# libjxl/jxl-rs

Measured on AMD Instinct MI355X. Metric: megapixels/sec decoded (8K VarDCT d1 reconstruction: dequant+CfL+IDCT+LF smoothing+Gaborish+EPF), higher is better.
Workload: dtype f32

## Files before the change

### jxl_rs_amd/csrc/k_filters_fused.hip

```cpp
#include "jxlh_internal.h"
#include "run_plan.h"

#ifndef JXLH_FUSED_TH
#define JXLH_FUSED_TH 56
#endif
#ifndef JXLH_FUSED_THREADS
#define JXLH_FUSED_THREADS 512
#endif
#ifndef JXLH_FUSED_TH_LOW
#define JXLH_FUSED_TH_LOW 24
#endif
#ifndef JXLH_FUSED_THREADS_LOW
#define JXLH_FUSED_THREADS_LOW 256
#endif
#ifndef JXLH_FUSED_WAVES_PER_EU
#define JXLH_FUSED_WAVES_PER_EU 6
#endif
#ifndef JXLH_FUSED_E0_WPE
#define JXLH_FUSED_E0_WPE 3
#endif
#ifndef JXLH_FUSED_E0_THREADS
#define JXLH_FUSED_E0_THREADS 128
#endif
#ifndef JXLH_SPARSE_MAX
#define JXLH_SPARSE_MAX 64
#endif
#ifndef JXLH_DENSE_ITEMS
#define JXLH_DENSE_ITEMS 40
#endif
#ifndef JXLH_DENSE_ITEMS0
#define JXLH_DENSE_ITEMS0 40
#endif

#ifndef JXLH_NT_FLOAD
#define JXLH_NT_FLOAD false
#endif
#ifndef JXLH_NT_FSTORE
#define JXLH_NT_FSTORE false
#endif
namespace jxlh {
namespace {

struct FusedArgs {
  const float* in[3];
  float* out[3];
  const float* inv_sigma;
  uint32_t stride, sigma_stride;
  int w, h;
  int y0, y1;
  float gab_k[3][3];
  float scale[3];
  float sm0, bsm0, sm1, bsm1, sm2, bsm2;
  int tiled_in, xblocks;
};

__device__ __forceinline__ uint32_t in_offset(const FusedArgs& a, int fx, int fy) {
  return 4u * (a.tiled_in ? ((uint32_t)((fy >> 3) * a.xblocks + (fx >> 3)) * 64u +
                             (uint32_t)((fy & 4) * 8 + (fx & 7) * 4 + (fy & 3)))
                          : ((uint32_t)fy * a.stride + (uint32_t)fx));
}
template <class T>
__device__ __forceinline__ const T& at_bytes(const float* base, uint32_t byte_off) {
  return *reinterpret_cast<const T*>(reinterpret_cast<const char*>(base) + byte_off);
}
template <class T>
__device__ __forceinline__ T& at_bytes(float* base, uint32_t byte_off) {
  return *reinterpret_cast<T*>(reinterpret_cast<char*>(base) + byte_off);
}

__device__ __forceinline__ float dpp_from_left(float v) {
  return __builtin_bit_cast(float, __builtin_amdgcn_update_dpp(0, __builtin_bit_cast(int, v), 0x111, 0xf, 0xf, true));
}
__device__ __forceinline__ float dpp_from_right(float v) {
  return __builtin_bit_cast(float, __builtin_amdgcn_update_dpp(0, __builtin_bit_cast(int, v), 0x101, 0xf, 0xf, true));
}

namespace tall {
#define JXLH_TILE_TH JXLH_FUSED_TH
#define JXLH_TILE_THREADS JXLH_FUSED_THREADS
#include "k_filters_fused_tile.inc"
#undef JXLH_TILE_TH
#undef JXLH_TILE_THREADS
}
namespace low {
#define JXLH_TILE_TH JXLH_FUSED_TH_LOW
#define JXLH_TILE_THREADS JXLH_FUSED_THREADS_LOW
#include "k_filters_fused_tile.inc"
#undef JXLH_TILE_TH
#undef JXLH_TILE_THREADS
}
using tall::recip_weight_sum;

__global__ void k_selftest_recip(uint32_t lo_bits, uint32_t hi_bits, unsigned long long* mismatches) {
  const uint32_t stride = gridDim.x * blockDim.x;
  unsigned long long bad = 0;
  for (uint64_t b = (uint64_t)lo_bits + blockIdx.x * blockDim.x + threadIdx.x; b < hi_bits; b += stride) {
    const float w = __builtin_bit_cast(float, (uint32_t)b);
    const float fast = recip_weight_sum(w);
    const float ref = 1.0f / w;
    bad += __builtin_bit_cast(uint32_t, fast) != __builtin_bit_cast(uint32_t, ref);
  }
  if (bad) atomicAdd(mismatches, bad);
}

}

void launch_selftest_recip(hipStream_t s, uint32_t lo_bits, uint32_t hi_bits, unsigned long long* mismatches) {
  hipLaunchKernelGGL(k_selftest_recip, dim3(2048), dim3(256), 0, s, lo_bits, hi_bits, mismatches);
}

int launch_fused_filters(hipStream_t s, const FrameDev& f, int y0, int y1) {
  const bool gab = f.gab != 0, e0 = f.epf_iters >= 3, e1 = f.epf_iters >= 1, e2 = f.epf_iters >= 2;
  const int where = StageList{gab, f.epf_iters, false}.fused_where();
  if (where == 0 || y1 <= y0) return where;
  FusedArgs a;
  for (int c = 0; c < 3; c++) {
    a.in[c] = f.planes[c];
    a.out[c] = f.tmp[c];
    a.scale[c] = f.epf_channel_scale[c];
    for (int k = 0; k < 3; k++) a.gab_k[c][k] = f.gab_k[c][k];
  }
  a.inv_sigma = f.inv_sigma;
  a.stride = (uint32_t)f.plane_stride;
  a.sigma_stride = (uint32_t)f.xblocks;
  a.w = f.xsize;
  a.h = f.ysize;
  a.y0 = y0;
  a.y1 = y1;
  a.sm0 = f.epf_sm[0];
  a.bsm0 = f.epf_bsm[0];
  a.sm1 = f.epf_sm[1];
  a.bsm1 = f.epf_bsm[1];
  a.sm2 = f.epf_sm[2];
  a.bsm2 = f.epf_bsm[2];
  a.tiled_in = f.tiled;
  a.xblocks = f.xblocks;
  if (e0) {
    a.y0 = max(0, y0 - 4);
    a.y1 = min(f.ysize, y1 + 3);
    if (gab) low::launch_variant<true, true, false, false>(s, a);
    else low::launch_variant<false, true, false, false>(s, a);
    for (int c = 0; c < 3; c++) {
      a.in[c] = f.tmp[c];
      a.out[c] = f.planes[c];
    }
    a.tiled_in = 0;
    a.y0 = y0;
    a.y1 = y1;
    tall::launch_variant<false, false, true, true>(s, a);
    return where;
  }
  if (gab && e1 && e2) low::launch_variant<true, false, true, true>(s, a);
  else if (gab && e1) low::launch_variant<true, false, true, false>(s, a);
  else if (gab) tall::launch_variant<true, false, false, false>(s, a);
  else if (e1 && e2) low::launch_variant<false, false, true, true>(s, a);
  else low::launch_variant<false, false, true, false>(s, a);
  return where;
}

}
```

### jxl_rs_amd/csrc/k_filters_fused_tile.inc

```
constexpr int kTW = 56, kTH = JXLH_TILE_TH, kB = 4;
constexpr int kBW = kTW + 2 * kB;
constexpr int kBH = kTH + 2 * kB;
constexpr int kStrips = kBW / 4;
constexpr int kPlane = kBW * kBH;
constexpr int kThreadsDefault = JXLH_TILE_THREADS;
static_assert(kStrips == 16, "lane <-> strip mapping relies on 16-lane DPP rows");
static_assert(kTH % 4 == 0 && kThreadsDefault % 64 == 0, "tiled staging fetches 4-row groups");
constexpr int kSigW = kBW / 8 + 2, kSigH = kBH / 8 + 2;
constexpr int kDenseItems = JXLH_DENSE_ITEMS, kDenseItems0 = JXLH_DENSE_ITEMS0, kSparseMax = JXLH_SPARSE_MAX;
static_assert(kSparseMax <= 64, "a compacting wavefront takes 64 strips");

#include "filters_core.inc"

template <int kT>
__device__ __forceinline__ void mirror_fill(float* __restrict__ buf, int m, int tx0, int ty0, int w, int h, int tid) {
  const int rw = kTW + 2 * m, rh = kTH + 2 * m;
  for (int idx = tid; idx < rw * rh; idx += kT) {
    const int bx = kB - m + idx % rw, by = kB - m + idx / rw;
    const int fx = tx0 - kB + bx, fy = ty0 - kB + by;
    if (fx >= 0 && fx < w && fy >= 0 && fy < h) continue;
    const int sx = mirror(fx, w) - (tx0 - kB), sy = mirror(fy, h) - (ty0 - kB);
    if (sx < 0 || sx >= kBW || sy < 0 || sy >= kBH) continue;
#pragma unroll
    for (int c = 0; c < 3; c++) buf[c * kPlane + by * kBW + bx] = buf[c * kPlane + sy * kBW + sx];
  }
}

template <bool E0>
constexpr int fused_threads() { return E0 ? JXLH_FUSED_E0_THREADS : kThreadsDefault; }

template <bool GAB, bool E0, bool E1, bool E2>
__global__ __launch_bounds__(fused_threads<E0>(), E0 ? JXLH_FUSED_E0_WPE : JXLH_FUSED_WAVES_PER_EU) void k23_fused_filters(const FusedArgs a) {
  constexpr int kT = fused_threads<E0>();
  __shared__ __attribute__((aligned(16))) float s_buf[3 * kPlane];
  __shared__ float s_sigma[kSigH * kSigW];
  __shared__ uint16_t s_list[(kTH + 2 * kB) * kStrips];
  __shared__ int s_cnt, s_nsw;
  const int tid_kernel = threadIdx.x, tid = tid_kernel;
  const int tiles_x = (a.w + kTW - 1) / kTW;
  const int tiles_y = (a.y1 - a.y0 + kTH - 1) / kTH;
  const int b = blockIdx.x, k = b & 7, j = b >> 3;
  const int tile_y = (j / tiles_x) * 8 + k, tile_x = j % tiles_x;
  if (tile_y >= tiles_y) return;
  constexpr int kBorder = (GAB ? 1 : 0) + (E0 ? 3 : 0) + (E1 ? 2 : 0) + (E2 ? 1 : 0);
  static_assert(kBorder >= 1 && kBorder <= kB, "at least one stage");
  static_assert(!(E0 && (E1 || E2)), "EPF0 closes its kernel; EPF1/EPF2 follow in a second launch");
  const int tx0 = tile_x * kTW;
  const int ty0 = a.y0 + tile_y * kTH;
  const bool edge = tx0 - kB < 0 || ty0 - kB < 0 || tx0 + kTW + kB > a.w || ty0 + kTH + kB > a.h;
  if (tid_kernel == 0) {
    s_cnt = 0;
    s_nsw = 0;
  }

  const int sbx0 = max(tx0 - kB, 0) >> 3, sby0 = max(ty0 - kB, 0) >> 3;
  if constexpr (E0 || E1 || E2) {
    if (tid < kSigH * kSigW) {
      const int sx = min(sbx0 + tid % kSigW, (a.w - 1) >> 3), sy = min(sby0 + tid / kSigW, (a.h - 1) >> 3);
      s_sigma[tid] = at_bytes<float>(a.inv_sigma, 4u * ((uint32_t)sy * a.sigma_stride + (uint32_t)sx));
    }
  }
  {
    constexpr int m = kBorder;
    constexpr int rows = kTH + 2 * m;
    if (!edge && a.tiled_in) {
      constexpr int yg0 = (kB - m) / 4, ygn = (rows + 2 * ((kB - m) % 4) + 3) / 4;
      constexpr int items = kBW * ((ygn + 1) / 2) * 2;
#pragma unroll
      for (int it = 0; it < (items + kT - 1) / kT; it++) {
        const int idx = it * kT + tid;
        const int w64 = idx >> 6, l = idx & 63;
        const int xh = w64 % 2, ypair = w64 / 2;
        const int bx = xh * 32 + (l & 31), yg = yg0 + ypair * 2 + (l >> 5);
        if (idx >= items || yg * 4 >= kBH) continue;
        const int by = yg * 4;
        const uint32_t off = in_offset(a, tx0 - kB + bx, ty0 - kB + by);
#pragma unroll
        for (int c = 0; c < 3; c++) {
          const float4 v = gload_f4<JXLH_NT_FLOAD>(&at_bytes<float>(a.in[c], off));
          float* d = s_buf + c * kPlane + by * kBW + bx;
          d[0] = v.x;
          d[kBW] = v.y;
          d[2 * kBW] = v.z;
          d[3 * kBW] = v.w;
        }
      }
    } else if (!edge) {
      for (int idx = tid; idx < kStrips * rows; idx += kT) {
        const int by = kB - m + idx / kStrips, bx0 = (idx % kStrips) * 4;
        const uint32_t off = in_offset(a, tx0 - kB + bx0, ty0 - kB + by);
#pragma unroll
        for (int c = 0; c < 3; c++)
          lds_store4(s_buf + c * kPlane + by * kBW + bx0, gload_f4<JXLH_NT_FLOAD>(&at_bytes<float>(a.in[c], off)));
      }
    } else {
      for (int idx = tid; idx < kStrips * rows; idx += kT) {
        const int by = kB - m + idx / kStrips, bx0 = (idx % kStrips) * 4;
        const int fy = mirror(ty0 - kB + by, a.h);
        const int fx0 = tx0 - kB + bx0;
        const int x0 = mirror(fx0, a.w), x1 = mirror(fx0 + 1, a.w), x2 = mirror(fx0 + 2, a.w),
                  x3 = mirror(fx0 + 3, a.w);
        const uint32_t o0 = in_offset(a, x0, fy), o1 = in_offset(a, x1, fy), o2 = in_offset(a, x2, fy),
                       o3 = in_offset(a, x3, fy);
#pragma unroll
        for (int c = 0; c < 3; c++) {
          const float* __restrict__ pl = a.in[c];
          lds_store4(s_buf + c * kPlane + by * kBW + bx0, make_float4(at_bytes<float>(pl, o0), at_bytes<float>(pl, o1), at_bytes<float>(pl, o2), at_bytes<float>(pl, o3)));
        }
      }
    }
  }
  __syncthreads();

  auto run_stage = [&](auto stage_tag, auto margin_tag) {
    constexpr int STAGE = decltype(stage_tag)::value;
    constexpr int margin = decltype(margin_tag)::value;
    constexpr bool last = margin == 0;
    constexpr int rows = kTH + 2 * margin;
    constexpr int n = (rows / 2) * kStrips;
    constexpr int kPasses = (n + kT - 1) / kT;
    static_assert(rows % 2 == 0, "4x2 items");
    int tid = tid_kernel;
    asm volatile("" : "+v"(tid));
    static_assert(STAGE != 3 || last, "EPF0 runs as the last stage");
    static_assert(STAGE != 2 || last, "EPF2 runs as the last stage");
    if constexpr (STAGE == 2 || STAGE == 3) {
      constexpr int ns = rows * kStrips;
      auto strip_geom = [&](int t, int& by, int& bx0, int& fy, int& fx0, float& sigma) {
        by = kB + t / kStrips;
        bx0 = (t % kStrips) * 4;
        fy = ty0 - kB + by;
        fx0 = tx0 - kB + bx0;
        const int sx = (min(max(fx0, 0), a.w - 1) >> 3) - sbx0, sy = (min(max(fy, 0), a.h - 1) >> 3) - sby0;
        sigma = s_sigma[sy * kSigW + sx];
      };
      auto store = [&](int bx0, int fy, int fx0, int c, float4 o) {
        if (bx0 >= kB && bx0 < kB + kTW && fy < a.y1 && fy < a.h && fx0 < a.w)
          gstore_f4<JXLH_NT_FSTORE>(&at_bytes<float>(a.out[c], 4u * ((uint32_t)fy * a.stride + (uint32_t)fx0)), o);
      };
#pragma unroll 1
      for (int t0 = 0; t0 < ns; t0 += kT) {
        if (t0 + (tid & ~63) >= ns) break;
        const int t = t0 + tid;
        const bool live = t < ns;
        int by, bx0, fy, fx0;
        float sigma;
        strip_geom(live ? t : 0, by, bx0, fy, fx0, sigma);
        const float* p = s_buf + by * kBW + bx0;
        auto put = [&](int c, float4 o) {
          if (live) store(bx0, fy, fx0, c, o);
        };
        const bool act = live && !(sigma < kMinSigma);
        const int cnt = __popcll(__ballot(act));
        if (cnt == 0) {
#pragma unroll
          for (int c = 0; c < 3; c++) put(c, lds_load4(p + c * kPlane));
        } else if (cnt >= (STAGE == 3 ? kDenseItems0 : kDenseItems)) {
          if constexpr (STAGE == 3) epf0_strip<false>(p, fx0, fy, sigma, a, put);
          else epf2_strip<false>(p, fx0, fy, sigma, a, put);
        } else {
          if (!act) {
#pragma unroll
            for (int c = 0; c < 3; c++) put(c, lds_load4(p + c * kPlane));
          } else {
            s_list[atomicAdd(&s_cnt, 1)] = (uint16_t)t;
          }
        }
      }
      {
        __syncthreads();
        const int cnt = s_cnt;
#pragma unroll 1
        for (int i0 = 0; i0 < cnt; i0 += kT) {
          if (i0 + (tid & ~63) >= cnt) break;
          const int i = i0 + tid;
          const bool on = i < cnt;
          const int t = s_list[min(i, cnt - 1)];
          int by, bx0, fy, fx0;
          float sigma;
          strip_geom(t, by, bx0, fy, fx0, sigma);
          const float* p = s_buf + by * kBW + bx0;
          auto put = [&](int c, float4 o) {
            if (on) store(bx0, fy, fx0, c, o);
          };
          if constexpr (STAGE == 3) epf0_strip<true>(p, fx0, fy, sigma, a, put, bx0 == 0, bx0 == kBW - 4);
          else epf2_strip<true>(p, fx0, fy, sigma, a, put, bx0 == 0, bx0 == kBW - 4);
        }
      }
      return;
    }
    static_assert(kPasses == 1 || STAGE == 0 || last, "held registers of one pass");
    auto geom_of = [&](int t) -> Geom {
      Geom g;
      g.live = t < n;
      const int by = kB - margin + (g.live ? (t / kStrips) * 2 : 0);
      g.bx0 = (t % kStrips) * 4;
      g.fy = ty0 - kB + by;
      g.fx0 = tx0 - kB + g.bx0;
      g.p = s_buf + by * kBW + g.bx0;
      if constexpr (STAGE != 0) {
        const int sx = (min(max(g.fx0, 0), a.w - 1) >> 3) - sbx0;
        const int sy0 = (min(max(g.fy, 0), a.h - 1) >> 3) - sby0, sy1 = (min(max(g.fy + 1, 0), a.h - 1) >> 3) - sby0;
        g.sigma0 = s_sigma[sy0 * kSigW + sx];
        g.sigma1 = s_sigma[sy1 * kSigW + sx];
      } else {
        g.sigma0 = g.sigma1 = 0.0f;
      }
      return g;
    };
    auto put_global = [&](const Geom& g, int r, int c, float4 o) {
      const int fyr = g.fy + r;
      if (g.live && g.bx0 >= kB && g.bx0 < kB + kTW && fyr < a.y1 && fyr < a.h && g.fx0 < a.w)
        gstore_f4<JXLH_NT_FSTORE>(&at_bytes<float>(a.out[c], 4u * ((uint32_t)fyr * a.stride + (uint32_t)g.fx0)), o);
    };
    float4 held[last ? 1 : kPasses][2][3];
    int held_e = -1;
    if constexpr (STAGE == 0) {
#pragma unroll
      for (int pass = 0; pass < kPasses; pass++) {
        if (pass * kT + (tid & ~63) >= n) continue;
        const Geom g = geom_of(pass * kT + tid);
        auto put_g = [&](int r, int c, float4 o) {
          if constexpr (last) put_global(g, r, c, o);
          else held[pass][r][c] = o;
        };
#pragma unroll
        for (int c = 0; c < 3; c++) gab_pair(g.p + c * kPlane, c, a.gab_k[c][0], a.gab_k[c][1], a.gab_k[c][2], put_g);
      }
    } else {
      static_assert(STAGE == 0 || STAGE == 3 || kPasses == 1, "one EPF item per thread (EPF0 returned above)");
      auto geom = [&]() -> Geom {
        int tl = tid_kernel;
        asm volatile("" : "+v"(tl));
        return geom_of(tl);
      };
      bool dense = false;
      int my_slot = -1;
      if ((tid & ~63) < n) {
        const Geom g = geom();
        const bool act0 = g.live && !(g.sigma0 < kMinSigma), act1 = g.live && !(g.sigma1 < kMinSigma);
        const unsigned long long m0 = __ballot(act0), m1 = __ballot(act1);
        const int cnt = __popcll(m0) + __popcll(m1);
        dense = cnt > kSparseMax;
        if (!dense) {
          int slot = 0, base = 0;
          if ((tid & 63) == 0) {
            slot = atomicAdd(&s_nsw, 1);
            if (cnt) base = atomicAdd(&s_cnt, cnt);
          }
          my_slot = __builtin_amdgcn_readfirstlane(slot);
          base = __builtin_amdgcn_readfirstlane(base);
          const unsigned long long below = (1ull << (tid & 63)) - 1ull;
          if (act0) s_list[base + __popcll(m0 & below)] = (uint16_t)(tid * 2);
          if (act1) s_list[base + __popcll(m0) + __popcll(m1 & below)] = (uint16_t)(tid * 2 + 1);
          if constexpr (last) {
#pragma unroll
            for (int r = 0; r < 2; r++) {
              if (r ? act1 : act0) continue;
#pragma unroll
              for (int c = 0; c < 3; c++) put_global(g, r, c, lds_load4(g.p + c * kPlane + r * kBW));
            }
          }
        }
      }
      __syncthreads();
      if (dense) {
        const Geom g = geom();
        auto put = [&](const Geom& gg, int r, int c, float4 o) {
          if constexpr (last) put_global(gg, r, c, o);
          else held[0][r][c] = o;
        };
        epf1_pair(g.p, geom, a, put);
        held_e = tid;
      } else if constexpr (STAGE == 1) {
        const int cnt = s_cnt;
        const int i = my_slot >= 0 ? my_slot * 64 + (tid & 63) : cnt;
        if (__any(i < cnt)) {
          const bool on = i < cnt;
          const int e = (int)s_list[min(i, cnt - 1)];
          const Geom g = geom_of(e >> 1);
          const int r = e & 1;
          epf1_strip_g(g.p + r * kBW, g.fx0, g.fy + r, r ? g.sigma1 : g.sigma0, g.bx0 == 0, g.bx0 == kBW - 4, a,
                       [&](int c, float4 o) {
                         if constexpr (last) {
                           if (on) put_global(g, r, c, o);
                         } else {
                           held[0][0][c] = o;
                         }
                       });
          if (on) held_e = e | 0x8000;
        }
      }
    }
    if constexpr (!last) {
      __syncthreads();
      if constexpr (STAGE == 0) {
#pragma unroll
        for (int pass = 0; pass < kPasses; pass++) {
          const int t = pass * kT + tid;
          if (t >= n) continue;
          float* d = s_buf + (kB - margin + (t / kStrips) * 2) * kBW + (t % kStrips) * 4;
#pragma unroll
          for (int r = 0; r < 2; r++)
#pragma unroll
            for (int c = 0; c < 3; c++) lds_store4(d + c * kPlane + r * kBW, held[pass][r][c]);
        }
      } else if (held_e >= 0) {
        const bool strip = (held_e & 0x8000) != 0;
        const int t = strip ? (held_e & 0x7fff) >> 1 : held_e, r0 = strip ? (held_e & 1) : 0;
        if (t < n) {
          float* d = s_buf + (kB - margin + (t / kStrips) * 2 + r0) * kBW + (t % kStrips) * 4;
#pragma unroll
          for (int c = 0; c < 3; c++) lds_store4(d + c * kPlane, held[0][0][c]);
          if (!strip) {
#pragma unroll
            for (int c = 0; c < 3; c++) lds_store4(d + c * kPlane + kBW, held[0][1][c]);
          }
        }
      }
      if constexpr (STAGE != 0) {
        if (tid == 0) {
          s_cnt = 0;
          s_nsw = 0;
        }
      }
      __syncthreads();
      if (edge) {
        mirror_fill<kT>(s_buf, margin, tx0, ty0, a.w, a.h, tid);
        __syncthreads();
      }
    }
  };
  constexpr int kMg = kBorder - (GAB ? 1 : 0);
  constexpr int kMe1 = kMg - (E1 ? 2 : 0);
  if constexpr (GAB) run_stage(std::integral_constant<int, 0>{}, std::integral_constant<int, kMg>{});
  if constexpr (E0) run_stage(std::integral_constant<int, 3>{}, std::integral_constant<int, 0>{});
  if constexpr (E1) run_stage(std::integral_constant<int, 1>{}, std::integral_constant<int, kMe1>{});
  if constexpr (E2) run_stage(std::integral_constant<int, 2>{}, std::integral_constant<int, 0>{});
}

template <bool GAB, bool E0, bool E1, bool E2>
void launch_variant(hipStream_t s, const FusedArgs& a) {
  const int tiles_x = (a.w + kTW - 1) / kTW, tiles_y = (a.y1 - a.y0 + kTH - 1) / kTH;
  const dim3 grid(tiles_x * ((tiles_y + 7) / 8) * 8);
  hipLaunchKernelGGL((k23_fused_filters<GAB, E0, E1, E2>), grid, dim3(fused_threads<E0>()), 0, s, a);
}
```

Baseline: 103,600.

## Build EPF work lists up front and skip EPF1 when tile is inactive

Moves sigma loading and the EPF1/closing-stage sparse/dense work-list construction to the kernel prologue, overlapping it with global loads held in registers before the LDS scatter. This removes per-stage ballot/atomic/list passes and one barrier per stage. When no EPF1 strip is active in a tile, Gaborish writes its result directly to global and the remaining stages are skipped. An optional profiling build mode is added. Holding the staged loads in registers raises register pressure, which may lower occupancy.

```diff
diff --git a/jxl_rs_amd/csrc/k_filters_fused.hip b/jxl_rs_amd/csrc/k_filters_fused.hip
--- a/jxl_rs_amd/csrc/k_filters_fused.hip
+++ b/jxl_rs_amd/csrc/k_filters_fused.hip
@@ -32,12 +32,71 @@
 #define JXLH_DENSE_ITEMS0 40
 #endif
 
+#ifndef JXLH_FUSED_GAB_DIRECT
+#define JXLH_FUSED_GAB_DIRECT 1
+#endif
+
 #ifndef JXLH_NT_FLOAD
 #define JXLH_NT_FLOAD false
 #endif
 #ifndef JXLH_NT_FSTORE
 #define JXLH_NT_FSTORE false
 #endif
+#ifdef JXLH_FUSED_PROF
+__device__ unsigned long long g_fused_prof[256][16];
+#define FPROF_DECL                                  \
+  __shared__ unsigned long long s_prof[16], s_prof_t; \
+  if (threadIdx.x == 0) {                           \
+    for (int i_ = 0; i_ < 16; i_++) s_prof[i_] = 0; \
+    s_prof[14] = 1;                                 \
+    s_prof_t = wall_clock64();                      \
+  }
+#define FPROF_MARK(i)                                    \
+  do {                                                   \
+    if (threadIdx.x == 0) {                              \
+      const unsigned long long now_ = wall_clock64();    \
+      s_prof[i] += now_ - s_prof_t;                      \
+      s_prof_t = now_;                                   \
+    }                                                    \
+  } while (0)
+#define FPROF_COUNT(i)                  \
+  do {                                  \
+    if (threadIdx.x == 0) s_prof[i]++;  \
+  } while (0)
+#define FPROF_FLUSH                                                                \
+  do {                                                                             \
+    if (threadIdx.x == 0)                                                          \
+      for (int i_ = 0; i_ < 16; i_++)                                              \
+        if (s_prof[i_]) atomicAdd(&g_fused_prof[blockIdx.x & 255][i_], s_prof[i_]); \
+  } while (0)
+#else
+#define FPROF_DECL
+#define FPROF_MARK(i) \
+  do {                \
+  } while (0)
+#define FPROF_COUNT(i) \
+  do {                 \
+  } while (0)
+#define FPROF_FLUSH \
+  do {              \
+  } while (0)
+#endif
+enum FusedPhase {
+  kPhLoads = 0,
+  kPhSigma = 1,
+  kPhLists = 2,
+  kPhScatter = 3,
+  kPhStaged = 4,
+  kPhGab = 5,
+  kPhGabBar = 6,
+  kPhGabWb = 7,
+  kPhE1 = 8,
+  kPhE1Bar = 9,
+  kPhE1Wb = 10,
+  kPhCloseOwn = 11,
+  kPhCloseList = 12,
+};
+
 namespace jxlh {
 namespace {
 
@@ -159,3 +218,21 @@
 }
 
 }
+
+#ifdef JXLH_FUSED_PROF
+extern "C" int jxlh_fused_prof_read(unsigned long long* out, int reset) {
+  static unsigned long long all[256][16];
+  if (out) {
+    if (hipMemcpyFromSymbol(all, HIP_SYMBOL(g_fused_prof), sizeof(all)) != hipSuccess) return -1;
+    for (int i = 0; i < 16; i++) {
+      out[i] = 0;
+      for (int k = 0; k < 256; k++) out[i] += all[k][i];
+    }
+  }
+  if (reset) {
+    memset(all, 0, sizeof all);
+    if (hipMemcpyToSymbol(HIP_SYMBOL(g_fused_prof), all, sizeof all) != hipSuccess) return -1;
+  }
+  return 0;
+}
+#endif
diff --git a/jxl_rs_amd/csrc/k_filters_fused_tile.inc b/jxl_rs_amd/csrc/k_filters_fused_tile.inc
--- a/jxl_rs_amd/csrc/k_filters_fused_tile.inc
+++ b/jxl_rs_amd/csrc/k_filters_fused_tile.inc
@@ -32,52 +32,161 @@
 template <bool GAB, bool E0, bool E1, bool E2>
 __global__ __launch_bounds__(fused_threads<E0>(), E0 ? JXLH_FUSED_E0_WPE : JXLH_FUSED_WAVES_PER_EU) void k23_fused_filters(const FusedArgs a) {
   constexpr int kT = fused_threads<E0>();
+  constexpr int kBorder = (GAB ? 1 : 0) + (E0 ? 3 : 0) + (E1 ? 2 : 0) + (E2 ? 1 : 0);
+  static_assert(kBorder >= 1 && kBorder <= kB, "at least one stage");
+  static_assert(!(E0 && (E1 || E2)), "EPF0 closes its kernel; EPF1/EPF2 follow in a second launch");
+  constexpr int kMg = kBorder - (GAB ? 1 : 0);
+  constexpr int kMe1 = kMg - (E1 ? 2 : 0);
+  constexpr bool kClose = E0 || E2;
+  constexpr int kN1 = ((kTH + 2 * kMe1) / 2) * kStrips, kWaves1 = (kN1 + 63) / 64;
+  constexpr int kNsC = kTH * kStrips, kPassesC = (kNsC + kT - 1) / kT;
+  constexpr int kDenseC = E0 ? kDenseItems0 : kDenseItems;
+  static_assert(!E1 || kN1 <= kT, "one EPF1 item per thread");
+  static_assert(kWaves1 < 64 && kPassesC <= 8, "bits of `plan`");
+  constexpr int kList1 = kWaves1 * kSparseMax;
+  constexpr int kPerWaveC = kDenseC - 1 < 64 ? (kDenseC - 1 > 0 ? kDenseC - 1 : 0) : 64;
+  constexpr int kListC = kPassesC * (kT / 64) * kPerWaveC < kNsC ? kPassesC * (kT / 64) * kPerWaveC : kNsC;
   __shared__ __attribute__((aligned(16))) float s_buf[3 * kPlane];
   __shared__ float s_sigma[kSigH * kSigW];
-  __shared__ uint16_t s_list[(kTH + 2 * kB) * kStrips];
-  __shared__ int s_cnt, s_nsw;
+  __shared__ uint16_t s_list1[E1 && kList1 > 0 ? kList1 : 1], s_listc[kClose && kListC > 0 ? kListC : 1];
+  __shared__ int s_cnt1, s_nsw1, s_cntc;
+  static_assert(kSigH * kSigW <= kT, "one 1/sigma per thread");
   const int tid_kernel = threadIdx.x, tid = tid_kernel;
   const int tiles_x = (a.w + kTW - 1) / kTW;
   const int tiles_y = (a.y1 - a.y0 + kTH - 1) / kTH;
   const int b = blockIdx.x, k = b & 7, j = b >> 3;
   const int tile_y = (j / tiles_x) * 8 + k, tile_x = j % tiles_x;
   if (tile_y >= tiles_y) return;
-  constexpr int kBorder = (GAB ? 1 : 0) + (E0 ? 3 : 0) + (E1 ? 2 : 0) + (E2 ? 1 : 0);
-  static_assert(kBorder >= 1 && kBorder <= kB, "at least one stage");
-  static_assert(!(E0 && (E1 || E2)), "EPF0 closes its kernel; EPF1/EPF2 follow in a second launch");
+  FPROF_DECL
   const int tx0 = tile_x * kTW;
   const int ty0 = a.y0 + tile_y * kTH;
   const bool edge = tx0 - kB < 0 || ty0 - kB < 0 || tx0 + kTW + kB > a.w || ty0 + kTH + kB > a.h;
   if (tid_kernel == 0) {
-    s_cnt = 0;
-    s_nsw = 0;
+    s_cnt1 = 0;
+    s_nsw1 = 0;
+    s_cntc = 0;
   }
 
   const int sbx0 = max(tx0 - kB, 0) >> 3, sby0 = max(ty0 - kB, 0) >> 3;
-  if constexpr (E0 || E1 || E2) {
-    if (tid < kSigH * kSigW) {
-      const int sx = min(sbx0 + tid % kSigW, (a.w - 1) >> 3), sy = min(sby0 + tid / kSigW, (a.h - 1) >> 3);
-      s_sigma[tid] = at_bytes<float>(a.inv_sigma, 4u * ((uint32_t)sy * a.sigma_stride + (uint32_t)sx));
-    }
-  }
-  {
-    constexpr int m = kBorder;
-    constexpr int rows = kTH + 2 * m;
-    if (!edge && a.tiled_in) {
-      constexpr int yg0 = (kB - m) / 4, ygn = (rows + 2 * ((kB - m) % 4) + 3) / 4;
-      constexpr int items = kBW * ((ygn + 1) / 2) * 2;
-#pragma unroll
-      for (int it = 0; it < (items + kT - 1) / kT; it++) {
-        const int idx = it * kT + tid;
-        const int w64 = idx >> 6, l = idx & 63;
-        const int xh = w64 % 2, ypair = w64 / 2;
-        const int bx = xh * 32 + (l & 31), yg = yg0 + ypair * 2 + (l >> 5);
-        if (idx >= items || yg * 4 >= kBH) continue;
-        const int by = yg * 4;
-        const uint32_t off = in_offset(a, tx0 - kB + bx, ty0 - kB + by);
+  __builtin_assume(tid >= 0 && tid < kT);
+  auto load_sigma = [&]() -> float {
+    const int i = min(tid, kSigH * kSigW - 1);
+    const int sx = min(sbx0 + i % kSigW, (a.w - 1) >> 3), sy = min(sby0 + i / kSigW, (a.h - 1) >> 3);
+    return at_bytes<float>(a.inv_sigma, 4u * ((uint32_t)sy * a.sigma_stride + (uint32_t)sx));
+  };
+
+  auto item_sigmas = [&](int t, bool live, float& sigma0, float& sigma1) {
+    const int by = kB - kMe1 + (live ? (t / kStrips) * 2 : 0);
+    const int fy = ty0 - kB + by, fx0 = tx0 - kB + (t % kStrips) * 4;
+    const int sx = (min(max(fx0, 0), a.w - 1) >> 3) - sbx0;
+    const int sy0 = (min(max(fy, 0), a.h - 1) >> 3) - sby0, sy1 = (min(max(fy + 1, 0), a.h - 1) >> 3) - sby0;
+    sigma0 = s_sigma[sy0 * kSigW + sx];
+    sigma1 = s_sigma[sy1 * kSigW + sx];
+  };
+  auto strip_sigma = [&](int t) -> float {
+    const int fy = ty0 + t / kStrips, fx0 = tx0 - kB + (t % kStrips) * 4;
+    const int sx = (min(max(fx0, 0), a.w - 1) >> 3) - sbx0, sy = (min(max(fy, 0), a.h - 1) >> 3) - sby0;
+    return s_sigma[sy * kSigW + sx];
+  };
+
+  auto build_lists = [&]() -> uint32_t {
+    uint32_t plan = 0;
+    const unsigned long long below = (1ull << (tid & 63)) - 1ull;
+    if constexpr (E1) {
+      if ((tid & ~63) < kN1) {
+        const bool live = tid < kN1;
+        float sigma0, sigma1;
+        item_sigmas(tid, live, sigma0, sigma1);
+        const bool act0 = live && !(sigma0 < kMinSigma), act1 = live && !(sigma1 < kMinSigma);
+        const unsigned long long m0 = __ballot(act0), m1 = __ballot(act1);
+        const int cnt = __popcll(m0) + __popcll(m1);
+        if (cnt > kSparseMax) {
+          plan |= 1u;
+        } else {
+          int slot = 0, base = 0;
+          if ((tid & 63) == 0) {
+            slot = atomicAdd(&s_nsw1, 1);
+            if (cnt) base = atomicAdd(&s_cnt1, cnt);
+          }
+          slot = __builtin_amdgcn_readfirstlane(slot);
+          base = __builtin_amdgcn_readfirstlane(base);
+          if (act0) s_list1[base + __popcll(m0 & below)] = (uint16_t)(tid * 2);
+          if (act1) s_list1[base + __popcll(m0) + __popcll(m1 & below)] = (uint16_t)(tid * 2 + 1);
+          plan |= (uint32_t)(slot + 1) << 1;
+        }
+      }
+    }
+    if constexpr (kClose) {
+#pragma unroll
+      for (int pass = 0; pass < kPassesC; pass++) {
+        if (pass * kT + (tid & ~63) >= kNsC) continue;
+        const int t = pass * kT + tid;
+        const bool act = t < kNsC && !(strip_sigma(t < kNsC ? t : 0) < kMinSigma);
+        const unsigned long long m = __ballot(act);
+        const int cnt = __popcll(m);
+        if (cnt == 0) continue;
+        if (cnt >= kDenseC) {
+          plan |= 1u << (8 + 2 * pass);
+        } else {
+          int base = 0;
+          if ((tid & 63) == 0) base = atomicAdd(&s_cntc, cnt);
+          base = __builtin_amdgcn_readfirstlane(base);
+          if (act) s_listc[base + __popcll(m & below)] = (uint16_t)t;
+          plan |= 2u << (8 + 2 * pass);
+        }
+      }
+    }
+    return __builtin_amdgcn_readfirstlane(plan);
+  };
+
+  constexpr int kStageRows = kTH + 2 * kBorder;
+  uint32_t plan = 0;
+  if (!edge) {
+    constexpr int kYg0 = (kB - kBorder) / 4, kYgn = (kStageRows + 2 * ((kB - kBorder) % 4) + 3) / 4;
+    constexpr int kItemsT = kBW * ((kYgn + 1) / 2) * 2, kItemsR = kStrips * kStageRows;
+    constexpr int kIt = ((kItemsT > kItemsR ? kItemsT : kItemsR) + kT - 1) / kT;
+    auto tiled_item = [&](int idx, int& bx, int& by) -> bool {
+      const int w64 = idx >> 6, l = idx & 63;
+      const int xh = w64 % 2, ypair = w64 / 2;
+      bx = xh * 32 + (l & 31);
+      by = (kYg0 + ypair * 2 + (l >> 5)) * 4;
+      return idx < kItemsT && by < kBH;
+    };
+    auto raster_item = [&](int idx, int& bx0, int& by) -> bool {
+      by = kB - kBorder + idx / kStrips;
+      bx0 = (idx % kStrips) * 4;
+      return idx < kItemsR;
+    };
+    const bool tiled = a.tiled_in != 0;
+    float sigma_in = 0.0f;
+    if constexpr (E0 || E1 || E2) sigma_in = load_sigma();
+    float4 staged[kIt][3];
+#pragma unroll
+    for (int it = 0; it < kIt; it++) {
+      int bxt, byt, bxr, byr;
+      const bool ont = tiled_item(it * kT + tid, bxt, byt), onr = raster_item(it * kT + tid, bxr, byr);
+      const bool on = tiled ? ont : onr;
+      const int bx = on ? (tiled ? bxt : bxr) : kB, by = on ? (tiled ? byt : byr) : kB;
+      const uint32_t off = in_offset(a, tx0 - kB + bx, ty0 - kB + by);
+#pragma unroll
+      for (int c = 0; c < 3; c++) staged[it][c] = gload_f4<JXLH_NT_FLOAD>(&at_bytes<float>(a.in[c], off));
+    }
+    FPROF_MARK(kPhLoads);
+    if constexpr (E0 || E1 || E2) {
+      if (tid < kSigH * kSigW) s_sigma[tid] = sigma_in;
+      __syncthreads();
+      FPROF_MARK(kPhSigma);
+      plan = build_lists();
+      FPROF_MARK(kPhLists);
+    }
+    if (tiled) {
+#pragma unroll
+      for (int it = 0; it < kIt; it++) {
+        int bx, by;
+        if (!tiled_item(it * kT + tid, bx, by)) continue;
 #pragma unroll
         for (int c = 0; c < 3; c++) {
-          const float4 v = gload_f4<JXLH_NT_FLOAD>(&at_bytes<float>(a.in[c], off));
+          const float4 v = staged[it][c];
           float* d = s_buf + c * kPlane + by * kBW + bx;
           d[0] = v.x;
           d[kBW] = v.y;
@@ -85,37 +194,46 @@
           d[3 * kBW] = v.w;
         }
       }
-    } else if (!edge) {
-      for (int idx = tid; idx < kStrips * rows; idx += kT) {
-        const int by = kB - m + idx / kStrips, bx0 = (idx % kStrips) * 4;
-        const uint32_t off = in_offset(a, tx0 - kB + bx0, ty0 - kB + by);
-#pragma unroll
-        for (int c = 0; c < 3; c++)
-          lds_store4(s_buf + c * kPlane + by * kBW + bx0, gload_f4<JXLH_NT_FLOAD>(&at_bytes<float>(a.in[c], off)));
-      }
     } else {
-      for (int idx = tid; idx < kStrips * rows; idx += kT) {
-        const int by = kB - m + idx / kStrips, bx0 = (idx % kStrips) * 4;
-        const int fy = mirror(ty0 - kB + by, a.h);
-        const int fx0 = tx0 - kB + bx0;
-        const int x0 = mirror(fx0, a.w), x1 = mirror(fx0 + 1, a.w), x2 = mirror(fx0 + 2, a.w),
-                  x3 = mirror(fx0 + 3, a.w);
-        const uint32_t o0 = in_offset(a, x0, fy), o1 = in_offset(a, x1, fy), o2 = in_offset(a, x2, fy),
-                       o3 = in_offset(a, x3, fy);
-#pragma unroll
-        for (int c = 0; c < 3; c++) {
-          const float* __restrict__ pl = a.in[c];
-          lds_store4(s_buf + c * kPlane + by * kBW + bx0, make_float4(at_bytes<float>(pl, o0), at_bytes<float>(pl, o1), at_bytes<float>(pl, o2), at_bytes<float>(pl, o3)));
-        }
+#pragma unroll
+      for (int it = 0; it < kIt; it++) {
+        int bx0, by;
+        if (!raster_item(it * kT + tid, bx0, by)) continue;
+#pragma unroll
+        for (int c = 0; c < 3; c++) lds_store4(s_buf + c * kPlane + by * kBW + bx0, staged[it][c]);
+      }
+    }
+  } else {
+    if constexpr (E0 || E1 || E2) {
+      const float sigma_in = load_sigma();
+      if (tid < kSigH * kSigW) s_sigma[tid] = sigma_in;
+      __syncthreads();
+      plan = build_lists();
+    }
+    for (int idx = tid; idx < kStrips * kStageRows; idx += kT) {
+      const int by = kB - kBorder + idx / kStrips, bx0 = (idx % kStrips) * 4;
+      const int fy = mirror(ty0 - kB + by, a.h);
+      const int fx0 = tx0 - kB + bx0;
+      const int x0 = mirror(fx0, a.w), x1 = mirror(fx0 + 1, a.w), x2 = mirror(fx0 + 2, a.w), x3 = mirror(fx0 + 3, a.w);
+      const uint32_t o0 = in_offset(a, x0, fy), o1 = in_offset(a, x1, fy), o2 = in_offset(a, x2, fy),
+                     o3 = in_offset(a, x3, fy);
+#pragma unroll
+      for (int c = 0; c < 3; c++) {
+        const float* __restrict__ pl = a.in[c];
+        lds_store4(s_buf + c * kPlane + by * kBW + bx0, make_float4(at_bytes<float>(pl, o0), at_bytes<float>(pl, o1), at_bytes<float>(pl, o2), at_bytes<float>(pl, o3)));
       }
     }
   }
+  FPROF_MARK(kPhScatter);
   __syncthreads();
-
-  auto run_stage = [&](auto stage_tag, auto margin_tag) {
+  FPROF_MARK(kPhStaged);
+
+  auto run_stage = [&](auto stage_tag, auto margin_tag, auto direct_tag) {
     constexpr int STAGE = decltype(stage_tag)::value;
     constexpr int margin = decltype(margin_tag)::value;
-    constexpr bool last = margin == 0;
+    constexpr bool direct = decltype(direct_tag)::value;
+    constexpr bool last = margin == 0 || direct;
+    static_assert(!direct || STAGE == 0, "only Gaborish computes a region wider than the tile");
     constexpr int rows = kTH + 2 * margin;
     constexpr int n = (rows / 2) * kStrips;
     constexpr int kPasses = (n + kT - 1) / kT;
@@ -126,20 +244,21 @@
     static_assert(STAGE != 2 || last, "EPF2 runs as the last stage");
     if constexpr (STAGE == 2 || STAGE == 3) {
       constexpr int ns = rows * kStrips;
+      static_assert(ns == kNsC, "the lists were built for this stage");
       auto strip_geom = [&](int t, int& by, int& bx0, int& fy, int& fx0, float& sigma) {
         by = kB + t / kStrips;
         bx0 = (t % kStrips) * 4;
         fy = ty0 - kB + by;
         fx0 = tx0 - kB + bx0;
-        const int sx = (min(max(fx0, 0), a.w - 1) >> 3) - sbx0, sy = (min(max(fy, 0), a.h - 1) >> 3) - sby0;
-        sigma = s_sigma[sy * kSigW + sx];
+        sigma = strip_sigma(t);
       };
       auto store = [&](int bx0, int fy, int fx0, int c, float4 o) {
         if (bx0 >= kB && bx0 < kB + kTW && fy < a.y1 && fy < a.h && fx0 < a.w)
           gstore_f4<JXLH_NT_FSTORE>(&at_bytes<float>(a.out[c], 4u * ((uint32_t)fy * a.stride + (uint32_t)fx0)), o);
       };
+      uint32_t forms = plan >> 8;
 #pragma unroll 1
-      for (int t0 = 0; t0 < ns; t0 += kT) {
+      for (int t0 = 0; t0 < ns; t0 += kT, forms >>= 2) {
         if (t0 + (tid & ~63) >= ns) break;
         const int t = t0 + tid;
         const bool live = t < ns;
@@ -150,32 +269,24 @@
         auto put = [&](int c, float4 o) {
           if (live) store(bx0, fy, fx0, c, o);
         };
-        const bool act = live && !(sigma < kMinSigma);
-        const int cnt = __popcll(__ballot(act));
-        if (cnt == 0) {
-#pragma unroll
-          for (int c = 0; c < 3; c++) put(c, lds_load4(p + c * kPlane));
-        } else if (cnt >= (STAGE == 3 ? kDenseItems0 : kDenseItems)) {
+        const int form = forms & 3;
+        if (form == 1) {
           if constexpr (STAGE == 3) epf0_strip<false>(p, fx0, fy, sigma, a, put);
           else epf2_strip<false>(p, fx0, fy, sigma, a, put);
-        } else {
-          if (!act) {
-#pragma unroll
-            for (int c = 0; c < 3; c++) put(c, lds_load4(p + c * kPlane));
-          } else {
-            s_list[atomicAdd(&s_cnt, 1)] = (uint16_t)t;
-          }
-        }
-      }
+        } else if (form == 0 || sigma < kMinSigma || !live) {
+#pragma unroll
+          for (int c = 0; c < 3; c++) put(c, lds_load4(p + c * kPlane));
+        }
+      }
+      FPROF_MARK(kPhCloseOwn);
       {
-        __syncthreads();
-        const int cnt = s_cnt;
+        const int cnt = s_cntc;
 #pragma unroll 1
         for (int i0 = 0; i0 < cnt; i0 += kT) {
           if (i0 + (tid & ~63) >= cnt) break;
           const int i = i0 + tid;
           const bool on = i < cnt;
-          const int t = s_list[min(i, cnt - 1)];
+          const int t = s_listc[min(i, cnt - 1)];
           int by, bx0, fy, fx0;
           float sigma;
           strip_geom(t, by, bx0, fy, fx0, sigma);
@@ -187,6 +298,7 @@
           else epf2_strip<true>(p, fx0, fy, sigma, a, put, bx0 == 0, bx0 == kBW - 4);
         }
       }
+      FPROF_MARK(kPhCloseList);
       return;
     }
     static_assert(kPasses == 1 || STAGE == 0 || last, "held registers of one pass");
@@ -199,10 +311,8 @@
       g.fx0 = tx0 - kB + g.bx0;
       g.p = s_buf + by * kBW + g.bx0;
       if constexpr (STAGE != 0) {
-        const int sx = (min(max(g.fx0, 0), a.w - 1) >> 3) - sbx0;
-        const int sy0 = (min(max(g.fy, 0), a.h - 1) >> 3) - sby0, sy1 = (min(max(g.fy + 1, 0), a.h - 1) >> 3) - sby0;
-        g.sigma0 = s_sigma[sy0 * kSigW + sx];
-        g.sigma1 = s_sigma[sy1 * kSigW + sx];
+        static_assert(STAGE != 1 || (margin == kMe1 && n == kN1), "the lists were built for this stage");
+        item_sigmas(t, g.live, g.sigma0, g.sigma1);
       } else {
         g.sigma0 = g.sigma1 = 0.0f;
       }
@@ -210,6 +320,9 @@
     };
     auto put_global = [&](const Geom& g, int r, int c, float4 o) {
       const int fyr = g.fy + r;
+      if constexpr (direct) {
+        if (fyr < ty0 || fyr >= ty0 + kTH) return;
+      }
       if (g.live && g.bx0 >= kB && g.bx0 < kB + kTW && fyr < a.y1 && fyr < a.h && g.fx0 < a.w)
         gstore_f4<JXLH_NT_FSTORE>(&at_bytes<float>(a.out[c], 4u * ((uint32_t)fyr * a.stride + (uint32_t)g.fx0)), o);
     };
@@ -229,41 +342,20 @@
       }
     } else {
       static_assert(STAGE == 0 || STAGE == 3 || kPasses == 1, "one EPF item per thread (EPF0 returned above)");
+      const int cnt = __builtin_amdgcn_readfirstlane(s_cnt1);
+      if constexpr (!last) {
+        if (cnt == 0 && __builtin_amdgcn_readfirstlane(s_nsw1) == kWaves1) {
+          if constexpr (!(GAB && JXLH_FUSED_GAB_DIRECT)) FPROF_COUNT(15);
+          return;
+        }
+      }
       auto geom = [&]() -> Geom {
         int tl = tid_kernel;
         asm volatile("" : "+v"(tl));
         return geom_of(tl);
       };
-      bool dense = false;
-      int my_slot = -1;
-      if ((tid & ~63) < n) {
-        const Geom g = geom();
-        const bool act0 = g.live && !(g.sigma0 < kMinSigma), act1 = g.live && !(g.sigma1 < kMinSigma);
-        const unsigned long long m0 = __ballot(act0), m1 = __ballot(act1);
-        const int cnt = __popcll(m0) + __popcll(m1);
-        dense = cnt > kSparseMax;
-        if (!dense) {
-          int slot = 0, base = 0;
-          if ((tid & 63) == 0) {
-            slot = atomicAdd(&s_nsw, 1);
-            if (cnt) base = atomicAdd(&s_cnt, cnt);
-          }
-          my_slot = __builtin_amdgcn_readfirstlane(slot);
-          base = __builtin_amdgcn_readfirstlane(base);
-          const unsigned long long below = (1ull << (tid & 63)) - 1ull;
-          if (act0) s_list[base + __popcll(m0 & below)] = (uint16_t)(tid * 2);
-          if (act1) s_list[base + __popcll(m0) + __popcll(m1 & below)] = (uint16_t)(tid * 2 + 1);
-          if constexpr (last) {
-#pragma unroll
-            for (int r = 0; r < 2; r++) {
-              if (r ? act1 : act0) continue;
-#pragma unroll
-              for (int c = 0; c < 3; c++) put_global(g, r, c, lds_load4(g.p + c * kPlane + r * kBW));
-            }
-          }
-        }
-      }
-      __syncthreads();
+      const bool dense = (plan & 1u) != 0;
+      const int my_slot = (int)((plan >> 1) & 0x7fu) - 1;
       if (dense) {
         const Geom g = geom();
         auto put = [&](const Geom& gg, int r, int c, float4 o) {
@@ -273,11 +365,21 @@
         epf1_pair(g.p, geom, a, put);
         held_e = tid;
       } else if constexpr (STAGE == 1) {
-        const int cnt = s_cnt;
+        if constexpr (last) {
+          if (my_slot >= 0) {
+            const Geom g = geom();
+#pragma unroll
+            for (int r = 0; r < 2; r++) {
+              if (g.live && !((r ? g.sigma1 : g.sigma0) < kMinSigma)) continue;
+#pragma unroll
+              for (int c = 0; c < 3; c++) put_global(g, r, c, lds_load4(g.p + c * kPlane + r * kBW));
+            }
+          }
+        }
         const int i = my_slot >= 0 ? my_slot * 64 + (tid & 63) : cnt;
         if (__any(i < cnt)) {
           const bool on = i < cnt;
-          const int e = (int)s_list[min(i, cnt - 1)];
+          const int e = (int)s_list1[min(i, cnt - 1)];
           const Geom g = geom_of(e >> 1);
           const int r = e & 1;
           epf1_strip_g(g.p + r * kBW, g.fx0, g.fy + r, r ? g.sigma1 : g.sigma0, g.bx0 == 0, g.bx0 == kBW - 4, a,
@@ -292,8 +394,10 @@
         }
       }
     }
+    FPROF_MARK(STAGE == 0 ? kPhGab : kPhE1);
     if constexpr (!last) {
       __syncthreads();
+      FPROF_MARK(STAGE == 0 ? kPhGabBar : kPhE1Bar);
       if constexpr (STAGE == 0) {
 #pragma unroll
         for (int pass = 0; pass < kPasses; pass++) {
@@ -318,25 +422,28 @@
           }
         }
       }
-      if constexpr (STAGE != 0) {
-        if (tid == 0) {
-          s_cnt = 0;
-          s_nsw = 0;
-        }
-      }
       __syncthreads();
       if (edge) {
         mirror_fill<kT>(s_buf, margin, tx0, ty0, a.w, a.h, tid);
         __syncthreads();
       }
+      FPROF_MARK(STAGE == 0 ? kPhGabWb : kPhE1Wb);
     }
   };
-  constexpr int kMg = kBorder - (GAB ? 1 : 0);
-  constexpr int kMe1 = kMg - (E1 ? 2 : 0);
-  if constexpr (GAB) run_stage(std::integral_constant<int, 0>{}, std::integral_constant<int, kMg>{});
-  if constexpr (E0) run_stage(std::integral_constant<int, 3>{}, std::integral_constant<int, 0>{});
-  if constexpr (E1) run_stage(std::integral_constant<int, 1>{}, std::integral_constant<int, kMe1>{});
-  if constexpr (E2) run_stage(std::integral_constant<int, 2>{}, std::integral_constant<int, 0>{});
+  constexpr std::false_type in_place{};
+  if constexpr (GAB && E1 && JXLH_FUSED_GAB_DIRECT) {
+    if (__builtin_amdgcn_readfirstlane(s_cnt1) == 0 && __builtin_amdgcn_readfirstlane(s_nsw1) == kWaves1) {
+      FPROF_COUNT(15);
+      run_stage(std::integral_constant<int, 0>{}, std::integral_constant<int, kMg>{}, std::true_type{});
+      FPROF_FLUSH;
+      return;
+    }
+  }
+  if constexpr (GAB) run_stage(std::integral_constant<int, 0>{}, std::integral_constant<int, kMg>{}, in_place);
+  if constexpr (E0) run_stage(std::integral_constant<int, 3>{}, std::integral_constant<int, 0>{}, in_place);
+  if constexpr (E1) run_stage(std::integral_constant<int, 1>{}, std::integral_constant<int, kMe1>{}, in_place);
+  if constexpr (E2) run_stage(std::integral_constant<int, 2>{}, std::integral_constant<int, 0>{}, in_place);
+  FPROF_FLUSH;
 }
 
 template <bool GAB, bool E0, bool E1, bool E2>
```

New measurement: 105,200, median of 6. No clear change (+1.5%).
